# kmaninis/OSVOS-PyTorch

Hardware: AMD Instinct MI355X
Metric: frames/sec (fwd+bwd) OSVOS-VGG16 854x480 per GPU; mask IoU vs ref (higher is better)
Workload: dtype f32 (3x bf16-split operands on MFMA, f32 accumulate); 1 GPU; 854x480 batch=1 online fine-tune loop (train_online.py), fused-head loss, nAveGrad=5, SGD 8-group, fp32x3, frame resident in HBM; global_batch=1, parallelism=dp1, grad_allreduce=none, rccl_ranks_seen=1

## Files before the change

### osvos-pytorch_amd/csrc/wgrad_f32x3.hip

```cpp
#include "common.h"
#include "kernels.h"
#include "h2split.h"

namespace {

typedef __bf16 bf16x8_t __attribute__((ext_vector_type(8)));
typedef __bf16 bf16x2_t __attribute__((ext_vector_type(2)));
typedef unsigned int u32x4 __attribute__((ext_vector_type(4)));
typedef short s16x4 __attribute__((ext_vector_type(4)));
typedef short s16x8 __attribute__((ext_vector_type(8)));
typedef __attribute__((address_space(3))) s16x4 lds_s16x4;

constexpr int PW = 16;

template <int PH_, int WAVES_, int S16_ = 0>
struct G3 {
  static constexpr int PH = PH_, WAVES = WAVES_, NT = 64 * WAVES_, S16 = S16_;
  static constexpr int BCO = S16_ ? 32 : 16 * WAVES_;
  static constexpr int BCI = S16_ ? 128 : 64;
  static constexpr int XOCT = BCI / 8;
  static constexpr int DYP = BCO * 2 + 64, XP = BCI * 2 + 64;
  static constexpr int PPIX = PW * PH, HW_ = PW + 2, XPIX = (PH + 2) * HW_;
  static constexpr int DY_B = PPIX * DYP, X_B = XPIX * XP;
  static constexpr int DOCT = BCO / 8;
  static constexpr int DY_ITEMS = PPIX * DOCT, X_ITEMS = XPIX * XOCT;
  static constexpr int DPG = NT / DOCT, XPG = NT / XOCT;
  static constexpr int NDY = (DY_ITEMS + NT - 1) / NT, NX = (X_ITEMS + NT - 1) / NT, NIT = NDY + NX;
  static constexpr int NST = 3 * PH;
  static constexpr int NB = WAVES_ == 8 ? 1 : 2;
  static constexpr size_t LDS = (size_t)3 * (DY_B + X_B);
  static_assert(NIT <= NST, "one staged item per stage must cover the patch");
  static_assert(LDS <= 160 * 1024, "tiles exceed the LDS of a CU");
};

struct W3Args {
  const void* x;
  const void* dy;
  float* slab;
  float* bslab;
  int N, H, W, Cin_s, Cout, Cout_s;
  int npx, npy, npatches, per_split, nco_t, nci_t;
  int map;
};

__device__ inline unsigned cvt2w(float a, float b) {
  bf16x2_t h;
  h[0] = (__bf16)a;
  h[1] = (__bf16)b;
  return __builtin_bit_cast(unsigned, h);
}
__device__ inline void split2w(float a, float b, unsigned& p0, unsigned& p1, unsigned& p2) {
  p0 = cvt2w(a, b);
  float ra = a - __uint_as_float(p0 << 16), rb = b - __uint_as_float(p0 & 0xffff0000u);
  p1 = cvt2w(ra, rb);
  ra -= __uint_as_float(p1 << 16);
  rb -= __uint_as_float(p1 & 0xffff0000u);
  p2 = cvt2w(ra, rb);
}
__device__ inline void split8w(const u32x4& lo, const u32x4& hi, u32x4& p0, u32x4& p1, u32x4& p2) {
  const f32x4 a = __builtin_bit_cast(f32x4, lo), b = __builtin_bit_cast(f32x4, hi);
  unsigned q0[4], q1[4], q2[4];
  split2w(a[0], a[1], q0[0], q1[0], q2[0]);
  split2w(a[2], a[3], q0[1], q1[1], q2[1]);
  split2w(b[0], b[1], q0[2], q1[2], q2[2]);
  split2w(b[2], b[3], q0[3], q1[3], q2[3]);
  p0 = u32x4{q0[0], q0[1], q0[2], q0[3]};
  p1 = u32x4{q1[0], q1[1], q1[2], q1[3]};
  p2 = u32x4{q2[0], q2[1], q2[2], q2[3]};
}

template <int NDS, int NVM, int NM = 18, int I = 0>
__device__ __forceinline__ void stage_groups() {
  if constexpr (I < NM) {
    __builtin_amdgcn_sched_group_barrier(0x008, 1, 0);
    constexpr int nds = (NDS * (I + 1)) / NM - (NDS * I) / NM, nvm = (NVM * (I + 1)) / NM - (NVM * I) / NM;
    if constexpr (nds > 0) __builtin_amdgcn_sched_group_barrier(0x100, nds, 0);
    if constexpr (nvm > 0) __builtin_amdgcn_sched_group_barrier(0x020, nvm, 0);
    __builtin_amdgcn_sched_group_barrier(0x006, 3, 0);
    stage_groups<NDS, NVM, NM, I + 1>();
  }
}

template <int PH, int WAVES, int S16 = 0, int ILV = 0, int NP = 3, int HP = 0, int OA = 0>
__global__ __launch_bounds__(64 * WAVES) void wgrad_f32x3_kernel(W3Args a) {
  static_assert(HP == 0 || NP == 2, "h2: two pieces");
  using G = G3<PH, WAVES, S16>;
  constexpr int NT = G::NT, BCO = G::BCO, BCI = G::BCI;
  extern __shared__ __attribute__((aligned(16))) char smem[];
  char* dYs = smem;
  char* Xs = smem + 3 * G::DY_B;
  const int tid = threadIdx.x, lane = tid & 63, wave = tid >> 6;
  const int wc = S16 ? 0 : wave >> 1, wi = S16 ? wave : wave & 1;
  constexpr unsigned OOB = 0x80000000u;

  int id = blockIdx.x;
  if (a.map == 1) id = (id & 7) * (gridDim.x >> 3) + (id >> 3);
  const int cit = id % a.nci_t;
  id /= a.nci_t;
  const int cot = id % a.nco_t;
  const int split = id / a.nco_t;
  const int co0 = cot * BCO, ci0 = cit * BCI;
  const int p_begin = split * a.per_split, p_end = min(p_begin + a.per_split, a.npatches);

  const int doct = tid % G::DOCT, dpg = tid / G::DOCT;
  const int xoct = tid % G::XOCT, xpg = tid / G::XOCT;
  const bool dy_ch_ok = co0 + 8 * doct < a.Cout, x_ch_ok = ci0 + 8 * xoct < a.Cin_s;
  u32x4 rdy[G::NDY][2], rx[G::NX][2];
  float bsum[8] = {0.f, 0.f, 0.f, 0.f, 0.f, 0.f, 0.f, 0.f};
  const bool want_bias = a.bslab != nullptr && cit == 0;
  const int img_dy_bytes = a.H * a.W * a.Cout_s * 4, img_x_bytes = a.H * a.W * a.Cin_s * 4;

  constexpr int DEADCOL = 0x40000000;
  unsigned dy_inv[G::NDY], x_inv[G::NX];
  unsigned dy_col[G::NDY], x_col[G::NX];
  if constexpr (OA == 0) {
#pragma unroll
    for (int it = 0; it < G::NDY; ++it) {
      const int p = dpg + G::DPG * it, py = p / PW, pxx = p - py * PW;
      const bool ok = dy_ch_ok && (G::DY_ITEMS % NT == 0 || p < G::PPIX);
      dy_inv[it] = (unsigned)(((py * a.W + pxx) * a.Cout_s + co0 + 8 * doct) * 4);
      dy_col[it] = (unsigned)(ok ? pxx : DEADCOL);
    }
#pragma unroll
    for (int j = 0; j < G::NX; ++j) {
      const int hp = xpg + G::XPG * j, hy = hp / G::HW_, hx = hp - hy * G::HW_;
      const bool ok = x_ch_ok && hp < G::XPIX;
      x_inv[j] = (unsigned)((((hy - 1) * a.W + hx - 1) * a.Cin_s + ci0 + 8 * xoct) * 4);
      x_col[j] = (unsigned)(ok ? hx - 1 : DEADCOL);
    }
  }

  struct Patch { __amdgpu_buffer_rsrc_t drs, xrs; int x0, y0; unsigned dorg, xorg; };
  auto locate = [&](int p, bool live) -> Patch {
    const int px = p % a.npx;
    int t = p / a.npx;
    const int py = t % a.npy;
    const int n = live ? t / a.npy : 0;
    Patch q;
    q.x0 = live ? px * PW : 0x40000000;
    q.y0 = py * PH;
    const unsigned org = (unsigned)(q.y0 * a.W + (live ? px * PW : 0));
    q.dorg = org * (unsigned)a.Cout_s * 4u;
    q.xorg = org * (unsigned)a.Cin_s * 4u;
    q.drs = __builtin_amdgcn_make_buffer_rsrc(const_cast<char*>(reinterpret_cast<const char*>(a.dy)) + (size_t)n * img_dy_bytes, 0, img_dy_bytes, 0x00020000);
    q.xrs = __builtin_amdgcn_make_buffer_rsrc(const_cast<char*>(reinterpret_cast<const char*>(a.x)) + (size_t)n * img_x_bytes, 0, img_x_bytes, 0x00020000);
    return q;
  };
  auto issue = [&](const Patch& q, int it) {
    if (it < G::NDY) {
      unsigned off;
      if constexpr (OA == 0) {
        off = (unsigned)q.x0 + dy_col[it] < (unsigned)a.W ? q.dorg + dy_inv[it] : OOB;
      } else {
        const int p = dpg + G::DPG * it, py = p / PW, pxx = p - py * PW;
        const bool ok = dy_ch_ok && (G::DY_ITEMS % NT == 0 || p < G::PPIX) && q.x0 + pxx < a.W;
        off = ok ? (unsigned)((((q.y0 + py) * a.W + q.x0 + pxx) * a.Cout_s + co0 + 8 * doct) * 4) : OOB;
      }
      rdy[it][0] = __builtin_amdgcn_raw_buffer_load_b128(q.drs, off, 0, 0);
      rdy[it][1] = __builtin_amdgcn_raw_buffer_load_b128(q.drs, off + 16u, 0, 0);
    } else if (it < G::NIT) {
      const int j = it - G::NDY;
      unsigned off;
      if constexpr (OA == 0) {
        off = (unsigned)q.x0 + x_col[j] < (unsigned)a.W ? q.xorg + x_inv[j] : OOB;
      } else {
        const int hp = xpg + G::XPG * j, hy = hp / G::HW_, hx = hp - hy * G::HW_;
        const bool ok = x_ch_ok && hp < G::XPIX && (unsigned)(q.x0 - 1 + hx) < (unsigned)a.W;
        off = ok ? (unsigned)((((q.y0 - 1 + hy) * a.W + q.x0 - 1 + hx) * a.Cin_s + ci0 + 8 * xoct) * 4) : OOB;
      }
      rx[j][0] = __builtin_amdgcn_raw_buffer_load_b128(q.xrs, off, 0, 0);
      rx[j][1] = __builtin_amdgcn_raw_buffer_load_b128(q.xrs, off + 16u, 0, 0);
    }
  };
  int h2_ed = kH2NoScale, h2_ex = kH2NoScale;
  float h2_sd = 1.f, h2_sx = 1.f;
  unsigned* const h2_mx = reinterpret_cast<unsigned*>(smem + G::LDS - 128);
  static_assert(HP == 0 || (G::X_B >= 128 && WAVES <= 8), "h2: exchange slots");
  auto store_patch = [&]() {
#pragma unroll
    for (int i = 0; i < G::NDY; ++i) {
      u32x4 p0, p1, p2;
      if (want_bias) {
        const f32x4 lo = __builtin_bit_cast(f32x4, rdy[i][0]), hi = __builtin_bit_cast(f32x4, rdy[i][1]);
#pragma unroll
        for (int c = 0; c < 4; ++c) { bsum[c] += lo[c]; bsum[4 + c] += hi[c]; }
      }
      if constexpr (HP != 0) h2_split8(rdy[i][0], rdy[i][1], h2_sd, p0, p1);
      else split8w(rdy[i][0], rdy[i][1], p0, p1, p2);
      const int p = dpg + G::DPG * i;
      if (G::DY_ITEMS % NT == 0 || p < G::PPIX) {
        char* d = dYs + p * G::DYP + doct * 16;
        *reinterpret_cast<u32x4*>(d) = p0;
        *reinterpret_cast<u32x4*>(d + G::DY_B) = p1;
        if constexpr (NP == 3) *reinterpret_cast<u32x4*>(d + 2 * G::DY_B) = p2;
      }
    }
#pragma unroll
    for (int j = 0; j < G::NX; ++j) {
      u32x4 p0, p1, p2;
      if constexpr (HP != 0) h2_split8(rx[j][0], rx[j][1], h2_sx, p0, p1);
      else split8w(rx[j][0], rx[j][1], p0, p1, p2);
      const int hp = xpg + G::XPG * j;
      if (G::X_ITEMS % NT == 0 || hp < G::XPIX) {
        char* d = Xs + hp * G::XP + xoct * 16;
        *reinterpret_cast<u32x4*>(d) = p0;
        *reinterpret_cast<u32x4*>(d + G::X_B) = p1;
        if constexpr (NP == 3) *reinterpret_cast<u32x4*>(d + 2 * G::X_B) = p2;
      }
    }
  };

  f32x16 acc[9];
#pragma unroll
  for (int t = 0; t < 9; ++t)
#pragma unroll
    for (int r = 0; r < 16; ++r) acc[t][r] = 0.f;

  const int fi = lane & 15, fg = (lane >> 4) & 1, lh = lane >> 5;
  const char* a_base = dYs + (8 * lh + (fi >> 2)) * G::DYP + (32 * wc + 16 * fg + 4 * (fi & 3)) * 2;
  const char* b_base = Xs + (8 * lh + (fi >> 2)) * G::XP + (32 * wi + 16 * fg + 4 * (fi & 3)) * 2;
  auto tr8 = [&](const char* p, int pitch) -> s16x8 {
    const s16x4 lo = __builtin_amdgcn_ds_read_tr16_b64_v4i16((lds_s16x4*)(p));
    const s16x4 hi = __builtin_amdgcn_ds_read_tr16_b64_v4i16((lds_s16x4*)(p + 4 * pitch));
    return __builtin_shufflevector(lo, hi, 0, 1, 2, 3, 4, 5, 6, 7);
  };

  {
    const Patch q = locate(p_begin, p_begin < p_end);
#pragma unroll
    for (int it = 0; it < G::NIT; ++it) issue(q, it);
  }
  for (int p = p_begin; p < p_end; ++p) {
    if constexpr (HP != 0) {
      unsigned md = 0, mxx = 0;
#pragma unroll
      for (int i = 0; i < G::NDY; ++i) md = h2_amax8(rdy[i][0], rdy[i][1], md);
#pragma unroll
      for (int j = 0; j < G::NX; ++j) mxx = h2_amax8(rx[j][0], rx[j][1], mxx);
      md = h2_wave_max(md);
      mxx = h2_wave_max(mxx);
      if (lane == 0) { h2_mx[(p & 1) * 16 + wave] = md; h2_mx[(p & 1) * 16 + 8 + wave] = mxx; }
    }
    __syncthreads();
    if constexpr (HP != 0) {
      const uint4* q = reinterpret_cast<const uint4*>(h2_mx) + (p & 1) * 4;
      const uint4 d0 = q[0], d1 = q[1], x0 = q[2], x1 = q[3];
      unsigned md = max(max(d0.x, d0.y), max(d0.z, d0.w)), mxx = max(max(x0.x, x0.y), max(x0.z, x0.w));
      if (WAVES == 8) { md = max(md, max(max(d1.x, d1.y), max(d1.z, d1.w))); mxx = max(mxx, max(max(x1.x, x1.y), max(x1.z, x1.w))); }
      const int ed = h2_exp(__builtin_amdgcn_readfirstlane(md)), ex = h2_exp(__builtin_amdgcn_readfirstlane(mxx));
      const int nd = ed < h2_ed ? ed : h2_ed, nx_ = ex < h2_ex ? ex : h2_ex;
      if (nd != h2_ed || nx_ != h2_ex) {
        const int dl = (h2_ed == kH2NoScale ? 0 : nd - h2_ed) + (h2_ex == kH2NoScale ? 0 : nx_ - h2_ex);
        if (dl != 0) {
#pragma unroll
          for (int t = 0; t < 9; ++t)
#pragma unroll
            for (int r = 0; r < 16; ++r) acc[t][r] = __builtin_ldexpf(acc[t][r], dl);
        }
        h2_ed = nd; h2_ex = nx_;
        h2_sd = h2_pow2(nd); h2_sx = h2_pow2(nx_);
      }
    }
    store_patch();
    __syncthreads();
    const Patch nx = locate(p + 1, p + 1 < p_end);
    constexpr int NB = G::NB;
    s16x8 af[NB][3], bfr[NB][3][3];
    auto lda = [&](int ks) {
#pragma unroll
      for (int pc = 0; pc < NP; ++pc) af[ks & (NB - 1)][pc] = tr8(a_base + pc * G::DY_B + ks * PW * G::DYP, G::DYP);
    };
    auto ldb = [&](int st) {
      const int ks = st / 3, r = st % 3;
#pragma unroll
      for (int pc = 0; pc < NP; ++pc)
#pragma unroll
        for (int s = 0; s < 3; ++s) bfr[st & (NB - 1)][pc][s] = tr8(b_base + pc * G::X_B + ((ks + r) * G::HW_ + s) * G::XP, G::XP);
    };
    if constexpr (NB == 2) {
      lda(0);
      ldb(0);
    }
#pragma unroll
    for (int st = 0; st < G::NST; ++st) {
      const int ks = st / 3, r = st % 3;
      if constexpr (NB == 2) {
        if (st + 1 < G::NST) {
          if (r == 2) lda(ks + 1);
          ldb(st + 1);
        }
      } else {
        if (r == 0) lda(ks);
        ldb(st);
      }
      issue(nx, st);
      if constexpr (ILV == 0) __builtin_amdgcn_sched_barrier(0);
      constexpr int NPROD = NP == 3 ? 6 : 3;
      constexpr int PX[6] = {NP == 3 ? 2 : 1, 0, NP == 3 ? 1 : 0, 1, 0, 0};
      constexpr int PD[6] = {0, NP == 3 ? 2 : 1, NP == 3 ? 1 : 0, 0, 1, 0};
#pragma unroll
      for (int t = 0; t < NPROD; ++t)
#pragma unroll
        for (int s = 0; s < 3; ++s)
          if constexpr (HP != 0)
            acc[r * 3 + s] = __builtin_amdgcn_mfma_f32_32x32x16_f16(__builtin_bit_cast(f16x8_t, bfr[st & (NB - 1)][PX[t]][s]),
                                                                   __builtin_bit_cast(f16x8_t, af[ks & (NB - 1)][PD[t]]), acc[r * 3 + s], 0, 0, 0);
          else
            acc[r * 3 + s] = __builtin_amdgcn_mfma_f32_32x32x16_bf16(__builtin_bit_cast(bf16x8_t, bfr[st & (NB - 1)][PX[t]][s]),
                                                                    __builtin_bit_cast(bf16x8_t, af[ks & (NB - 1)][PD[t]]), acc[r * 3 + s], 0, 0, 0);
      if constexpr (ILV != 0) {
        constexpr int V = 2;
        const bool last = st + 1 >= G::NST, wide = r == 2, vm = st < G::NIT;
        constexpr int NM = 3 * NPROD, DN = 6 * NP, DW = 8 * NP;
        if (last) { if (vm) stage_groups<0, V, NM>(); else stage_groups<0, 0, NM>(); }
        else if (wide) { if (vm) stage_groups<DW, V, NM>(); else stage_groups<DW, 0, NM>(); }
        else { if (vm) stage_groups<DN, V, NM>(); else stage_groups<DN, 0, NM>(); }
      }
      __builtin_amdgcn_sched_barrier(0);
    }
  }
  __syncthreads();
  if constexpr (HP != 0) {
    const int dl = (h2_ed == kH2NoScale || h2_ex == kH2NoScale) ? 0 : -(h2_ed + h2_ex);
#pragma unroll
    for (int t = 0; t < 9; ++t)
#pragma unroll
      for (int r = 0; r < 16; ++r) acc[t][r] = __builtin_ldexpf(acc[t][r], dl);
  }

  {
    const int li = lane & 31;
    const size_t slab_elems = (size_t)9 * a.Cout * a.Cin_s;
    const __amdgpu_buffer_rsrc_t srs = __builtin_amdgcn_make_buffer_rsrc(a.slab + (size_t)split * slab_elems, 0, (int)(slab_elems * 4), 0x00020000);
    const int co = co0 + wc * 32 + li;
    const int cib = ci0 + wi * 32 + 4 * lh;
    const unsigned row = co < a.Cout ? (unsigned)(co * a.Cin_s) * 4u : OOB;
    const unsigned tap_stride = (unsigned)(a.Cout * a.Cin_s) * 4u;
#pragma unroll
    for (int t = 0; t < 9; ++t)
#pragma unroll
      for (int q = 0; q < 4; ++q) {
        const int ci = cib + 8 * q;
        const unsigned off = ci < a.Cin_s ? row + (unsigned)t * tap_stride + (unsigned)ci * 4u : OOB;
        const f32x4 v = {acc[t][4 * q], acc[t][4 * q + 1], acc[t][4 * q + 2], acc[t][4 * q + 3]};
        __builtin_amdgcn_raw_buffer_store_b128(__builtin_bit_cast(u32x4, v), srs, off, 0, 0);
      }
  }
  if (want_bias) {
    float* red = reinterpret_cast<float*>(smem);
#pragma unroll
    for (int c = 0; c < 8; ++c) red[dpg * BCO + doct * 8 + c] = bsum[c];
    __syncthreads();
    if (tid < BCO) {
      float sum = 0.f;
      for (int g = 0; g < G::DPG; ++g) sum += red[g * BCO + tid];
      if (co0 + tid < a.Cout) a.bslab[(size_t)split * a.Cout + co0 + tid] = sum;
    }
  }
}

void plan3(int N, int H, int W, int Cin_s, int Cout, WgradPlan* p) {
  *p = WgradPlan();
  p->family = WGRAD_F32X3;
  if (Cout == 16) {
    p->nci_t = ceil_div(Cin_s, 128);
    wgrad_patches(p, N, H, W, PW, 4);
  } else {
    p->nco_t = ceil_div(Cout, 64);
    p->nci_t = ceil_div(Cin_s, 64);
    wgrad_patches(p, N, H, W, PW, (ceil_div(H, 6) * 6 <= ceil_div(H, 4) * 4) ? 6 : 4);
  }
  wgrad_split(p, 256, 2, 256, (size_t)9 * Cout * Cin_s, Cout);
  OSVOS_ENV_INT(map_env, "OSVOS_WGRAD_MAP", 1);
  p->map = (map_env == 1 && p->blocks % 8 == 0) ? 1 : 0;
  p->reduce = osvos_wgrad_reduce_kind(p->nsplit, Cout, Cin_s, Cin_s);
}

template <int PH, int WAVES, int S16 = 0, int ILV = 0, int NP = 3, int HP = 0, int OA = 0>
int launch3(const W3Args& a, long blocks, hipStream_t stream) {
  constexpr size_t lds = G3<PH, WAVES, S16>::LDS;
  if (int rc = osvos_set_dyn_lds_once<&wgrad_f32x3_kernel<PH, WAVES, S16, ILV, NP, HP, OA>>(lds)) return rc;
  hipLaunchKernelGGL((wgrad_f32x3_kernel<PH, WAVES, S16, ILV, NP, HP, OA>), dim3((unsigned)blocks), dim3(64 * WAVES), lds, stream, a);
  OSVOS_LAUNCH_CHECK();
  return 0;
}

typedef int (*W3Launch)(const W3Args&, long, hipStream_t);
constexpr W3Launch kKernels[] = {
    launch3<4, 4, 1, 1, 2, 0, 1>, launch3<6, 4, 0, 1, 2, 0, 1>, launch3<4, 4, 0, 1, 2, 0, 1>,
    launch3<4, 4, 1, 1, 3, 0, 1>, launch3<6, 4, 0, 1, 3, 0, 1>, launch3<4, 4, 0, 1, 3, 0, 1>,
    launch3<4, 4, 1, 1, 2, 1>,    launch3<6, 4, 0, 1, 2, 1>,    launch3<4, 4, 0, 1, 2, 1>,
    launch3<4, 4, 1, 1, 2>,       launch3<6, 4, 0, 1, 2>,       launch3<4, 4, 0, 1, 2>,
    launch3<4, 4, 1, 1>,          launch3<6, 4, 0, 1>,          launch3<4, 4, 0, 1>,
};
enum { FORM_OLD2 = 0, FORM_OLD3 = 1, FORM_H2 = 2, FORM_X2 = 3, FORM_X3 = 4 };

int choose(const WgradCall& c, WgradPlan* p) {
  OSVOS_ARG_CHECK(c.x && c.dy && c.ws && c.dw, "wgrad f32x3: null pointer");
  OSVOS_ARG_CHECK(c.N > 0 && c.H > 0 && c.W > 0, "wgrad f32x3: bad shape");
  const bool skinny = osvos_wgrad_f32x3_skinny_applicable(c);
  OSVOS_ARG_CHECK(skinny || osvos_wgrad_f32x3_wide_applicable(c),
                  "wgrad f32x3: unsupported shape (Cin %d/%d Cout %d/%d)", c.Cin, c.Cin_s, c.Cout, c.Cout_s);
  OSVOS_ARG_CHECK((long)c.H * c.W * c.Cin_s < (1L << 28) && (long)c.H * c.W * c.Cout_s < (1L << 28), "wgrad f32x3: image too large for 31-bit byte offsets");
  OSVOS_ARG_CHECK(!c.x_bf16 && !c.dy_bf16, "wgrad f32x3: fp32 tensors only");
  plan3(c.N, c.H, c.W, c.Cin_s, c.Cout, p);
  const bool two = c.pieces == 2;
  const bool h2 = c.pieces == 22;
  OSVOS_ENV_INT(oldaddr_env, "OSVOS_WGRAD_X3_OLDADDR", 0);
  const bool oa = oldaddr_env == 1 && !h2;
  const int form = oa ? (two ? FORM_OLD2 : FORM_OLD3) : h2 ? FORM_H2 : two ? FORM_X2 : FORM_X3;
  p->kernel = 3 * form + (skinny ? 0 : p->ph == 6 ? 1 : 2);
  return 0;
}

}

bool osvos_wgrad_f32x3_wide_applicable(const WgradCall& c) {
  return c.Cin == c.Cin_s && c.Cin_s % 64 == 0 && c.Cout % 64 == 0 && c.Cout_s % 4 == 0;
}
bool osvos_wgrad_f32x3_skinny_applicable(const WgradCall& c) {
  return c.Cout == 16 && c.Cout_s == 16 && c.Cin == c.Cin_s && c.Cin_s % 128 == 0;
}

size_t osvos_wgrad_f32x3_ws_bytes(int N, int H, int W, int Cin_s, int Cout) {
  if (!osvos_wgrad_f32x3_applicable(wgrad_shape_call(N, H, W, Cin_s, Cout))) return 0;
  WgradPlan p;
  plan3(N, H, W, Cin_s, Cout, &p);
  return wgrad_plan_ws_bytes(p);
}

int osvos_wgrad_f32x3_plan(const WgradCall& c, WgradPlan* p) { return choose(c, p); }

int osvos_conv3x3_wgrad_f32x3(const WgradCall& c) {
  WgradPlan p;
  if (int rc = choose(c, &p)) return rc;
  W3Args a;
  a.x = c.x; a.dy = c.dy;
  a.slab = reinterpret_cast<float*>(c.ws);
  a.bslab = c.db ? a.slab + p.slab_floats : nullptr;
  a.N = c.N; a.H = c.H; a.W = c.W; a.Cin_s = c.Cin_s; a.Cout = c.Cout; a.Cout_s = c.Cout_s;
  a.npx = p.npx; a.npy = p.npy; a.npatches = p.npatches; a.per_split = p.per_split; a.nco_t = p.nco_t; a.nci_t = p.nci_t;
  a.map = p.map;
  if (c.phase != WGRAD_REDUCE)
    if (int rc = kKernels[p.kernel](a, p.blocks, c.stream)) return rc;
  if (c.phase == WGRAD_PARTIALS) return 0;
  return osvos_wgrad_reduce_launch(p.reduce, a.slab, a.bslab, c.dw, c.db, p.nsplit, c.Cout, c.Cin, c.Cin_s, c.accumulate, c.stream);
}
```

Baseline: 253.1 frames/s.

## Add dedicated 16-output-channel wgrad kernel with 8-wave cin tiling and LDS transpose reads

```diff
diff --git a/osvos-pytorch_amd/csrc/wgrad_f32x3.hip b/osvos-pytorch_amd/csrc/wgrad_f32x3.hip
--- a/osvos-pytorch_amd/csrc/wgrad_f32x3.hip
+++ b/osvos-pytorch_amd/csrc/wgrad_f32x3.hip
@@ -359,6 +359,159 @@
   }
 }
 
+template <int PH_>
+struct GT {
+  static constexpr int PH = PH_, NT = 512, BCI = 128, NBLK = BCI / 16;
+  static constexpr int PPIX = PW * PH, HW_ = PW + 2, XPIX = (PH + 2) * HW_;
+  static constexpr int PB = 32;
+  static constexpr int DY_B = PPIX * PB;
+  static constexpr int XB_B = XPIX * PB + 32;
+  static constexpr int X_B = NBLK * XB_B;
+  static constexpr int NX = (XPIX * (BCI / 8) + NT - 1) / NT;
+  static constexpr size_t LDS = (size_t)3 * (DY_B + X_B);
+  static_assert(PH % 2 == 0, "a k-step is two patch rows");
+  static_assert(2 * PPIX <= NT, "one dY item per thread");
+  static_assert(NBLK * 64 == NT, "one wave per 16-cin block");
+  static_assert(PPIX * 16 * 4 <= LDS, "bias partials reuse the tiles");
+};
+
+template <int PH>
+__global__ __launch_bounds__(512, 2) void wgrad_f32x3_t16_kernel(W3Args a) {
+  using G = GT<PH>;
+  extern __shared__ __attribute__((aligned(16))) char smem[];
+  char* dYs = smem;
+  char* Xs = smem + 3 * G::DY_B;
+  const int tid = threadIdx.x, lane = tid & 63, wave = tid >> 6;
+  constexpr unsigned OOB = 0x80000000u;
+
+  int id = blockIdx.x;
+  if (a.map == 1) id = (id & 7) * (gridDim.x >> 3) + (id >> 3);
+  const int cit = id % a.nci_t, split = id / a.nci_t;
+  const int ci0 = cit * G::BCI;
+  const int p_begin = split * a.per_split, p_end = min(p_begin + a.per_split, a.npatches);
+
+  const bool dy_thr = tid < 2 * G::PPIX;
+  const int doct = tid & 1, dpix = tid >> 1, dpy = dpix / PW, dpx = dpix % PW;
+  const int xoct = tid & 15, xpg = tid >> 4;
+  u32x4 rdy[2], rx[G::NX][2];
+  float bsum[8] = {0.f, 0.f, 0.f, 0.f, 0.f, 0.f, 0.f, 0.f};
+  const bool want_bias = a.bslab != nullptr && cit == 0;
+  const int img_dy_bytes = a.H * a.W * 16 * 4, img_x_bytes = a.H * a.W * a.Cin_s * 4;
+
+  auto issue = [&](int p, bool live) {
+    const int px = p % a.npx;
+    const int t = p / a.npx;
+    const int py = t % a.npy, n = live ? t / a.npy : 0;
+    const int x0 = px * PW, y0 = py * PH;
+    const __amdgpu_buffer_rsrc_t drs = __builtin_amdgcn_make_buffer_rsrc(const_cast<char*>(reinterpret_cast<const char*>(a.dy)) + (size_t)n * img_dy_bytes, 0, img_dy_bytes, 0x00020000);
+    const __amdgpu_buffer_rsrc_t xrs = __builtin_amdgcn_make_buffer_rsrc(const_cast<char*>(reinterpret_cast<const char*>(a.x)) + (size_t)n * img_x_bytes, 0, img_x_bytes, 0x00020000);
+    {
+      const bool ok = live && dy_thr && x0 + dpx < a.W;
+      const unsigned off = ok ? (unsigned)((((y0 + dpy) * a.W + x0 + dpx) * 16 + 8 * doct) * 4) : OOB;
+      rdy[0] = __builtin_amdgcn_raw_buffer_load_b128(drs, off, 0, 0);
+      rdy[1] = __builtin_amdgcn_raw_buffer_load_b128(drs, off + 16u, 0, 0);
+    }
+#pragma unroll
+    for (int j = 0; j < G::NX; ++j) {
+      const int hp = xpg + (G::NT / 16) * j, hy = hp / G::HW_, hx = hp - hy * G::HW_;
+      const bool ok = live && hp < G::XPIX && (unsigned)(x0 - 1 + hx) < (unsigned)a.W;
+      const unsigned off = ok ? (unsigned)((((y0 - 1 + hy) * a.W + x0 - 1 + hx) * a.Cin_s + ci0 + 8 * xoct) * 4) : OOB;
+      rx[j][0] = __builtin_amdgcn_raw_buffer_load_b128(xrs, off, 0, 0);
+      rx[j][1] = __builtin_amdgcn_raw_buffer_load_b128(xrs, off + 16u, 0, 0);
+    }
+  };
+  auto store_patch = [&]() {
+    if (dy_thr) {
+      if (want_bias) {
+        const f32x4 lo = __builtin_bit_cast(f32x4, rdy[0]), hi = __builtin_bit_cast(f32x4, rdy[1]);
+#pragma unroll
+        for (int c = 0; c < 4; ++c) { bsum[c] += lo[c]; bsum[4 + c] += hi[c]; }
+      }
+      u32x4 p0, p1, p2;
+      split8w(rdy[0], rdy[1], p0, p1, p2);
+      char* d = dYs + dpix * G::PB + doct * 16;
+      *reinterpret_cast<u32x4*>(d) = p0;
+      *reinterpret_cast<u32x4*>(d + G::DY_B) = p1;
+      *reinterpret_cast<u32x4*>(d + 2 * G::DY_B) = p2;
+    }
+#pragma unroll
+    for (int j = 0; j < G::NX; ++j) {
+      const int hp = xpg + (G::NT / 16) * j;
+      if (hp < G::XPIX) {
+        u32x4 p0, p1, p2;
+        split8w(rx[j][0], rx[j][1], p0, p1, p2);
+        char* d = Xs + (xoct >> 1) * G::XB_B + hp * G::PB + (xoct & 1) * 16;
+        *reinterpret_cast<u32x4*>(d) = p0;
+        *reinterpret_cast<u32x4*>(d + G::X_B) = p1;
+        *reinterpret_cast<u32x4*>(d + 2 * G::X_B) = p2;
+      }
+    }
+  };
+
+  f32x4 acc[9];
+#pragma unroll
+  for (int t = 0; t < 9; ++t) acc[t] = f32x4{0.f, 0.f, 0.f, 0.f};
+
+  const int fi = lane & 15, kg = lane >> 4;
+  const char* a_base = dYs + (4 * kg + (fi >> 2)) * G::PB + (fi & 3) * 8;
+  const char* b_base = Xs + wave * G::XB_B + (4 * kg + (fi >> 2)) * G::PB + (fi & 3) * 8;
+  auto tr8 = [&](const char* up, const char* dn) -> bf16x8_t {
+    const s16x4 lo = __builtin_amdgcn_ds_read_tr16_b64_v4i16((lds_s16x4*)(up));
+    const s16x4 hi = __builtin_amdgcn_ds_read_tr16_b64_v4i16((lds_s16x4*)(dn));
+    return __builtin_bit_cast(bf16x8_t, __builtin_shufflevector(lo, hi, 0, 1, 2, 3, 4, 5, 6, 7));
+  };
+
+  issue(p_begin, p_begin < p_end);
+  for (int p = p_begin; p < p_end; ++p) {
+    __syncthreads();
+    store_patch();
+    __syncthreads();
+    issue(p + 1, p + 1 < p_end);
+#pragma unroll 1
+    for (int ks = 0; ks < PH / 2; ++ks) {
+      bf16x8_t af[3];
+#pragma unroll
+      for (int pc = 0; pc < 3; ++pc) af[pc] = tr8(a_base + pc * G::DY_B + (2 * ks) * PW * G::PB, a_base + pc * G::DY_B + (2 * ks + 1) * PW * G::PB);
+#pragma unroll
+      for (int r = 0; r < 3; ++r)
+#pragma unroll
+        for (int s = 0; s < 3; ++s) {
+          bf16x8_t bfr[3];
+#pragma unroll
+          for (int pc = 0; pc < 3; ++pc)
+            bfr[pc] = tr8(b_base + pc * G::X_B + ((2 * ks + r) * G::HW_ + s) * G::PB, b_base + pc * G::X_B + ((2 * ks + 1 + r) * G::HW_ + s) * G::PB);
+          constexpr int PX[6] = {2, 0, 1, 1, 0, 0};
+          constexpr int PD[6] = {0, 2, 1, 0, 1, 0};
+#pragma unroll
+          for (int t = 0; t < 6; ++t) acc[r * 3 + s] = __builtin_amdgcn_mfma_f32_16x16x32_bf16(bfr[PX[t]], af[PD[t]], acc[r * 3 + s], 0, 0, 0);
+          if (s == 2) __builtin_amdgcn_sched_barrier(0);
+        }
+    }
+  }
+  __syncthreads();
+
+  {
+    const size_t slab_elems = (size_t)9 * 16 * a.Cin_s;
+    const __amdgpu_buffer_rsrc_t srs = __builtin_amdgcn_make_buffer_rsrc(a.slab + (size_t)split * slab_elems, 0, (int)(slab_elems * 4), 0x00020000);
+    const unsigned at = (unsigned)(fi * a.Cin_s + ci0 + 16 * wave + 4 * kg) * 4u, tap_stride = (unsigned)(16 * a.Cin_s) * 4u;
+#pragma unroll
+    for (int t = 0; t < 9; ++t) __builtin_amdgcn_raw_buffer_store_b128(__builtin_bit_cast(u32x4, acc[t]), srs, at + (unsigned)t * tap_stride, 0, 0);
+  }
+  if (want_bias) {
+    float* red = reinterpret_cast<float*>(smem);
+    if (dy_thr) {
+#pragma unroll
+      for (int c = 0; c < 8; ++c) red[dpix * 16 + doct * 8 + c] = bsum[c];
+    }
+    __syncthreads();
+    if (tid < 16) {
+      float sum = 0.f;
+      for (int g = 0; g < G::PPIX; ++g) sum += red[g * 16 + tid];
+      a.bslab[(size_t)split * 16 + tid] = sum;
+    }
+  }
+}
+
 void plan3(int N, int H, int W, int Cin_s, int Cout, WgradPlan* p) {
   *p = WgradPlan();
   p->family = WGRAD_F32X3;
@@ -376,6 +529,15 @@
   p->reduce = osvos_wgrad_reduce_kind(p->nsplit, Cout, Cin_s, Cin_s);
 }
 
+template <int PH>
+int launch_t16(const W3Args& a, long blocks, hipStream_t stream) {
+  constexpr size_t lds = GT<PH>::LDS;
+  if (int rc = osvos_set_dyn_lds_once<&wgrad_f32x3_t16_kernel<PH>>(lds)) return rc;
+  hipLaunchKernelGGL((wgrad_f32x3_t16_kernel<PH>), dim3((unsigned)blocks), dim3(GT<PH>::NT), lds, stream, a);
+  OSVOS_LAUNCH_CHECK();
+  return 0;
+}
+
 template <int PH, int WAVES, int S16 = 0, int ILV = 0, int NP = 3, int HP = 0, int OA = 0>
 int launch3(const W3Args& a, long blocks, hipStream_t stream) {
   constexpr size_t lds = G3<PH, WAVES, S16>::LDS;
@@ -388,10 +550,10 @@
 typedef int (*W3Launch)(const W3Args&, long, hipStream_t);
 constexpr W3Launch kKernels[] = {
     launch3<4, 4, 1, 1, 2, 0, 1>, launch3<6, 4, 0, 1, 2, 0, 1>, launch3<4, 4, 0, 1, 2, 0, 1>,
-    launch3<4, 4, 1, 1, 3, 0, 1>, launch3<6, 4, 0, 1, 3, 0, 1>, launch3<4, 4, 0, 1, 3, 0, 1>,
+    launch_t16<4>,                launch3<6, 4, 0, 1, 3, 0, 1>, launch3<4, 4, 0, 1, 3, 0, 1>,
     launch3<4, 4, 1, 1, 2, 1>,    launch3<6, 4, 0, 1, 2, 1>,    launch3<4, 4, 0, 1, 2, 1>,
     launch3<4, 4, 1, 1, 2>,       launch3<6, 4, 0, 1, 2>,       launch3<4, 4, 0, 1, 2>,
-    launch3<4, 4, 1, 1>,          launch3<6, 4, 0, 1>,          launch3<4, 4, 0, 1>,
+    launch_t16<4>,                launch3<6, 4, 0, 1>,          launch3<4, 4, 0, 1>,
 };
 enum { FORM_OLD2 = 0, FORM_OLD3 = 1, FORM_H2 = 2, FORM_X2 = 3, FORM_X3 = 4 };
 
@@ -403,11 +565,11 @@
                   "wgrad f32x3: unsupported shape (Cin %d/%d Cout %d/%d)", c.Cin, c.Cin_s, c.Cout, c.Cout_s);
   OSVOS_ARG_CHECK((long)c.H * c.W * c.Cin_s < (1L << 28) && (long)c.H * c.W * c.Cout_s < (1L << 28), "wgrad f32x3: image too large for 31-bit byte offsets");
   OSVOS_ARG_CHECK(!c.x_bf16 && !c.dy_bf16, "wgrad f32x3: fp32 tensors only");
-  plan3(c.N, c.H, c.W, c.Cin_s, c.Cout, p);
   const bool two = c.pieces == 2;
   const bool h2 = c.pieces == 22;
   OSVOS_ENV_INT(oldaddr_env, "OSVOS_WGRAD_X3_OLDADDR", 0);
   const bool oa = oldaddr_env == 1 && !h2;
+  plan3(c.N, c.H, c.W, c.Cin_s, c.Cout, p);
   const int form = oa ? (two ? FORM_OLD2 : FORM_OLD3) : h2 ? FORM_H2 : two ? FORM_X2 : FORM_X3;
   p->kernel = 3 * form + (skinny ? 0 : p->ph == 6 ? 1 : 2);
   return 0;
```

Measured after the change: 254.7 frames/s (median of 6 runs). About the same (+0.6%).
